# dfdazac/grapes

Measured on AMD Instinct MI355X. Metric: sampled edges aggregated/sec, ogbn-products 3-layer GFlowNet, higher is better.
Workload: dtype f32

## Files before the change

### grapes_amd/_lib.py

```python
from __future__ import annotations

import ctypes as C
import os

_HERE = os.path.dirname(os.path.abspath(__file__))
DIAG_LIB_PATH = os.path.join(_HERE, "libgrapes_hip_diag.so")
DIAG = os.environ.get("GRAPES_DIAG", "0") == "1"
LIB_PATH = os.environ.get("GRAPES_LIB_PATH") or (DIAG_LIB_PATH if DIAG else os.path.join(_HERE, "libgrapes_hip.so"))
ABI_MAJOR, ABI_MINOR = 3, 2


def diag_switch(name: str, default: str) -> str:
    if os.environ.get("GRAPES_DIAG", "0") == "1":
        return os.environ.get(name, default)
    return default


P = C.c_void_p
I32 = C.c_int32
I64 = C.c_int64
U32 = C.c_uint32
U64 = C.c_uint64
F32 = C.c_float
SZ = C.c_size_t
# ... 66 lines not shown
    "grapes_frontier_offsets": (I32, [P, P, I32, P, P, P, P]),
    "grapes_frontier_expand": (I32, [P, P, P, I32, P, P, I32, P, P, P, P, P]),
    "grapes_frontier_expand_fused": (I32, [P, P, P, I32, P, I32, P, P, P, P, P, P, P, I32, P, P, P, P, P]),
    "grapes_frontier_expand_fused_ext": (I32, [P, P, P, I32, P, I32, P, P, P, P, P, P, P, I32, P, P, P, P, P, P, P, P, P]),
    "grapes_slice_stage_words": (SZ, [I32]),
    "grapes_bitmap_mark": (I32, [P, P, P, I64, P, I32, P, P]),
    "grapes_bitmap_mark_rows": (I32, [P, P, P, I32, P, P, I32, P, P]),
    "grapes_bitmap_clear": (I32, [P, P, I64, P, P]),
    "grapes_frontier_compact_workspace_bytes": (SZ, [I32, I32]),
    "grapes_frontier_compact": (I32, [P, P, P, I32, I32, P, P, P, P, P, P, U32, P, I32, P, P, SZ, P, SZ, P, SZ, P, P, P, P, P]),
    "grapes_frontier_compact_counted": (I32, [P, P, P, I32, I32, P, P, P, P, P, P, U32, P, I32, P, P, SZ, P, SZ, P, SZ, P, P, P, P, P, P]),
    "grapes_gcn_prepare_counted": (I32, [P, P, P, I32, P, P, I32, P, P, P, P, P, P, P, P, P, P, P, P, P, I64, I32, P, P]),
    "grapes_bitmap_mark_hop": (I32, [P, P, P, P, I32, P, P, P, I32, P, I32, P, P]),
    "grapes_bitmap_mark_lists": (I32, [P, P, P, I32, P, P, I32, P, P, I32, P, P, I32, P, I32, P, P, P]),
    "grapes_union_sorted": (I32, [P, I32, P, P, I32, P, P, I32, P, P, I32, P, I32, I32, P, P, P, P, P, P]),
    "grapes_slice_mark": (I32, [P, P, I32, P, I32, P, P]),
    "grapes_slice_remark": (I32, [P, P, I32, P, P, I32, P, P, P, I32, P, P]),
    "grapes_slice_filter_workspace_bytes": (SZ, [I32]),
    "grapes_slice_filter": (I32, [P, P, P, I32, P, I32, P, P, P, P, P, I32, P, P]),
    "grapes_indicator_mark": (I32, [P, P, I32, P, U32, P, I32, I32, P]),
    "grapes_step_begin": (I32, [P, P, I32, P, I32, P, I32, I32, I32, P, P, I32, I32, P, P]),
    "grapes_gather_rows": (I32, [P, I32, P, I32, P, P, U32, P, I32, P, P]),
    "grapes_gcn_prepare_workspace_bytes": (SZ, [I32, I32]),
    "grapes_gcn_prepare_zero_words": (SZ, [I32]),
    "grapes_gcn_long_items_capacity": (I32, [I32]),
    "grapes_gcn_prepare": (I32, [P, P, I32, P, P, I32, P, I32, P, P, P, P, P, P, P, P, P, P, P, P, P]),
    "grapes_gcn_prepare_prefetching": (I32, [P, P, I32, P, P, I32, P, I32, P, P, P, P, P, P, P, P, P, P, P, P, P, I64, I32, P]),
    "grapes_gcn_prepare_small_batch": (I32, [I32, P, P, P, P, P, I32, P, P, P, P, P, P, P, P, P, P, P, P, P, P, P, P]),
    "grapes_gcn_prepare_from_csr": (I32, [P, I32, P, P, P, I32, P]),
    "grapes_linear_fwd": (I32, [P, P, P, I32, P, I32, I32, P]),
# ... 143 lines not shown
```

### grapes_amd/csrc/index_kernels.hip

```cpp
#include "common.h"

__global__ void tensormap_update_k(int32_t* __restrict__ map, const int32_t* __restrict__ keys,
                                   int n_host, const int32_t* d_n) {
    const int n = eff_count(d_n, n_host);
    for (int i = blockIdx.x * blockDim.x + threadIdx.x; i < n; i += gridDim.x * blockDim.x)
        map[keys[i]] = i;
}

__global__ void tensormap_map_k(const int32_t* __restrict__ map, const int32_t* __restrict__ keys,
                                int32_t* __restrict__ out, int64_t n_host, const int32_t* d_n) {
    int64_t n = n_host;
    if (d_n) { int64_t v = *d_n; n = v < n_host ? v : n_host; }
    for (int64_t i = (int64_t)blockIdx.x * blockDim.x + threadIdx.x; i < n;
         i += (int64_t)gridDim.x * blockDim.x)
        out[i] = map[keys[i]];
}

extern "C" int grapes_tensormap_update(int32_t* map, const int32_t* keys, int32_t n,
                                       const int32_t* d_n, grapes_stream_t stream) {
    if (!map || (!keys && n > 0) || n < 0) return GRAPES_EINVAL;
    if (n == 0) return 0;
    int grid = grapes_div_up(n, 256); if (grid > 2048) grid = 2048;
    hipLaunchKernelGGL(tensormap_update_k, dim3(grid), dim3(256), 0, (hipStream_t)stream, map, keys, n, d_n);
    GRAPES_LAUNCH_CHECK();
// ... 703 lines not shown
    bool overflow = false;
    for (int i = lo; i < hi; ++i) {
        const int v = key[i];
        if (v != 0x7fffffff && (i == 0 || key[i - 1] != v)) {
            if (pos < n_cap) { out_ids[pos] = v; if (node_map) node_map[v] = pos; }
            else overflow = true;
            if (unmark_mult) unmark_mult[v] = 0;
            ++pos;
        }
    }
    if (tid == 0) { counts[0] = tot < n_cap ? tot : n_cap; counts[1] = counts[0]; }
    if (overflow && status) atomicOr(status, GRAPES_STATUS_NODE_OVERFLOW);
    (void)s_total;
}

__global__ __launch_bounds__(1024) void union_sorted_k(MarkLists L, int num_nodes, int n_cap, int32_t* __restrict__ out_ids,
                                                       int32_t* __restrict__ node_map, int32_t* __restrict__ counts,
                                                       int32_t* __restrict__ unmark_mult, int32_t* status) {
    union_sorted_body(L, num_nodes, n_cap, out_ids, node_map, counts, unmark_mult, status);
}

extern "C" int grapes_bitmap_clear(uint64_t* bits, const int32_t* ids, int64_t n, const int32_t* d_n,
                                   grapes_stream_t stream) {
    if (!bits || (!ids && n > 0) || n < 0) return GRAPES_EINVAL;
    if (n == 0) return 0;
    int grid = grapes_div_up(n, 256); if (grid > 4096) grid = 4096;
    hipLaunchKernelGGL(bitmap_clear_k, dim3(grid), dim3(256), 0, (hipStream_t)stream,
                       (unsigned long long*)bits, ids, n, d_n);
    GRAPES_LAUNCH_CHECK();
    return 0;
}

__device__ __forceinline__ int block_prefix_of_sums(const int32_t* __restrict__ bsum, int b, int* lds) {
    int acc = 0;
// ... 252 lines not shown
};
#define COMPACT_EMIT_CALL(A, bid, nblk)                                                                                              \
    compact_emit_body((A).bits, (A).prev_bits, (A).W, (A).bsum_b, (A).bsum_n, (A).n_cap, (A).batch_nodes, (A).neighbor_nodes,          \
                      (A).nb_local, (A).node_map, (A).counts, (A).status, (A).ind_code, (A).epoch_host, (A).d_epoch, (A).ind_bit,      \
                      (A).sync, (A).cand_pos, (A).zero_a, (A).words_a, (A).zero_b, (A).words_b, (A).zero_c, (A).words_c, (A).rm,       \
                      (A).gc, (A).hd, bid, nblk)
__global__ __launch_bounds__(1024) void compact_emit_k(CompactEmitArgs a) { COMPACT_EMIT_CALL(a, (int)blockIdx.x, (int)gridDim.x); }
__global__ __launch_bounds__(1024) void compact_emit_pair_k(CompactEmitArgs a, CompactEmitArgs b, int nA) {
    if ((int)blockIdx.x < nA) COMPACT_EMIT_CALL(a, (int)blockIdx.x, nA);
    else COMPACT_EMIT_CALL(b, (int)blockIdx.x - nA, (int)gridDim.x - nA);
}

__global__ __launch_bounds__(1024) void union_sorted_compact_pair_k(MarkLists L, int num_nodes, int n_cap, int32_t* __restrict__ out_ids,
                                                                   int32_t* __restrict__ node_map, int32_t* __restrict__ counts,
                                                                   int32_t* __restrict__ unmark_mult, int32_t* status,
                                                                   CompactEmitArgs b) {
    if (blockIdx.x == 0) union_sorted_body(L, num_nodes, n_cap, out_ids, node_map, counts, unmark_mult, status);
    else COMPACT_EMIT_CALL(b, (int)blockIdx.x - 1, (int)gridDim.x - 1);
}

extern "C" int grapes_union_sorted(const int32_t* ids0, int32_t n0, const int32_t* d_n0, const int32_t* ids1, int32_t n1,
                                   const int32_t* d_n1, const int32_t* ids2, int32_t n2, const int32_t* d_n2,
                                   const int32_t* ids3, int32_t n3, const int32_t* d_n3, int32_t num_nodes, int32_t n_cap,
                                   int32_t* out_ids, int32_t* node_map, int32_t* counts, int32_t* unmark_mult,
                                   int32_t* status, grapes_stream_t stream) {
    if (n0 < 0 || n1 < 0 || n2 < 0 || n3 < 0 || num_nodes <= 0 || n_cap <= 0 || !out_ids || !counts) return GRAPES_EINVAL;
    if ((long long)n0 + n1 + n2 + n3 > UNION_MAX) return GRAPES_EINVAL;
    MarkLists L{{n0 > 0 ? ids0 : nullptr, n1 > 0 ? ids1 : nullptr, n2 > 0 ? ids2 : nullptr, n3 > 0 ? ids3 : nullptr},
                {n0, n1, n2, n3}, {d_n0, d_n1, d_n2, d_n3}};
    if (const GrapesRiderRecord* r = grapes_rider_match(GRAPES_RK_COMPACT, 0, 1024, (hipStream_t)stream)) {
        CompactEmitArgs Bq; memcpy(&Bq, r->args, sizeof Bq);
        hipLaunchKernelGGL(union_sorted_compact_pair_k, dim3(1 + r->grid), dim3(1024), 0, (hipStream_t)stream, L, num_nodes, n_cap, out_ids,
                           node_map, counts, unmark_mult, status, Bq);
    } else {
        hipLaunchKernelGGL(union_sorted_k, dim3(1), dim3(1024), 0, (hipStream_t)stream, L, num_nodes, n_cap, out_ids, node_map, counts,
                           unmark_mult, status);
    }
    GRAPES_LAUNCH_CHECK();
    return 0;
}


template <int WPT>
__global__ __launch_bounds__(1024) void compact_emit_wide_k(unsigned long long* __restrict__ bits,
                                                            const unsigned long long* __restrict__ prev_bits, int W,
                                                            int n_cap, int32_t* __restrict__ batch_nodes,
                                                            int32_t* __restrict__ neighbor_nodes, int32_t* __restrict__ nb_local,
                                                            int32_t* __restrict__ node_map, int32_t* __restrict__ counts,
                                                            int32_t* status, uint32_t* __restrict__ ind_code,
                                                            uint32_t epoch_host, const uint32_t* d_epoch, int ind_bit,
                                                            unsigned long long* __restrict__ sync, int32_t* __restrict__ cand_pos,
                                                            uint32_t* __restrict__ zero_a, size_t words_a,
                                                            uint32_t* __restrict__ zero_b, size_t words_b,
                                                            uint32_t* __restrict__ zero_c, size_t words_c,
// ... 793 lines not shown
```

### grapes_amd/csrc/prep_kernels.hip

```cpp
#include "common.h"

struct PrefetchRows { const float* X; long long pitch; int row_floats; const int32_t* ids; int32_t* sink; };
__device__ __forceinline__ void prefetch_rows_body(const PrefetchRows& pf, int n, int block, int nblocks) {
    const int spr = (pf.row_floats * 4 + 63) / 64;
    const long long total = (long long)n * spr;
    unsigned acc = 0u;
    for (long long i = (long long)block * blockDim.x + threadIdx.x; i < total; i += (long long)nblocks * blockDim.x) {
        const int r = (int)(i / spr), k = (int)(i - (long long)r * spr);
        int c = 16 * k; if (c > pf.row_floats - 1) c = pf.row_floats - 1;
        acc += __float_as_uint(pf.X[(long long)pf.ids[r] * pf.pitch + c]);
    }
    if (acc == 0x7fc12345u && pf.sink) *pf.sink = 1;
}


__global__ void prep_hist_k(const int32_t* __restrict__ es, const int32_t* __restrict__ ed, int e_host,
                            const int32_t* d_e, int n_host, const int32_t* d_n, int grouped,
                            int32_t* __restrict__ cnt_t, int32_t* __restrict__ cnt_s,
                            int32_t* __restrict__ seg_first, int32_t* __restrict__ seg_last,
                            int32_t* __restrict__ loops, int32_t* __restrict__ nseg, int32_t* __restrict__ bad,
                            int32_t* status, const int32_t* __restrict__ relabel, int32_t* __restrict__ n_long,
                            int ge, PrefetchRows pf) {
    const int e = eff_count(d_e, e_host);
    const int n = eff_count(d_n, n_host);
// ... 504 lines not shown
                            int32_t* __restrict__ rl_dst, int32_t* __restrict__ counters, size_t counter_words,
                            int32_t* __restrict__ csr_dst, int clear_dst, int32_t* __restrict__ n_long) {
    const int e = eff_count(d_e, e_host);
    if (n_long && blockIdx.x == 0 && threadIdx.x < 2) n_long[threadIdx.x] = 0;
    const size_t stride = (size_t)gridDim.x * blockDim.x;
    const size_t i0 = (size_t)blockIdx.x * blockDim.x + threadIdx.x;
    for (size_t i = i0; i < counter_words; i += stride) counters[i] = 0;
    for (size_t t = i0; t < (size_t)e_host; t += stride) {
        if (clear_dst) csr_dst[t] = 0;
        if (node_map && t < (size_t)e) { rl_src[t] = node_map[es[t]]; rl_dst[t] = node_map[ed[t]]; }
    }
}

#define SMALL_N 2048
#define SMALL_T 1024
__device__ __forceinline__ int slice_assemble(const int32_t* __restrict__ stage, int fe_cap, const int32_t* d_fe, int out_cap,
                                              int32_t* __restrict__ out_src, int32_t* __restrict__ out_dst, int32_t* d_out_count,
                                              int32_t* status, int* lds) {
    const int tid = threadIdx.x;
    const int fe = eff_count(d_fe, fe_cap);
    const int nwb_cap = (fe_cap + 63) >> 6, nwb = (fe + 63) >> 6;
    const int32_t* wcnt = stage; const int32_t* wsum = stage + nwb_cap;
    const int32_t* st_s = stage + 2 * nwb_cap; const int32_t* st_d = st_s + fe_cap; const int32_t* st_c = st_d + fe_cap;
    const int per = (nwb + SMALL_T - 1) / SMALL_T;
    const int w0 = tid * per;
    int mine = 0;
    for (int k = 0; k < per; ++k) { const int wb = w0 + k; if (wb < nwb) mine += wsum[wb]; }
    int tot;
    int pos = block_excl_scan(mine, lds, &tot);
    bool overflow = false;
    if (mine > 0) {
        for (int k = 0; k < per; ++k) {
            const int wb = w0 + k;
            if (wb >= nwb) break;
            const int cnt = wcnt[wb];
            for (int i = 0; i < cnt; ++i) {
                const int q = wb * 64 + i;
                const int sv = st_s[q], dv = st_d[q], c = st_c[q];
                for (int r = 0; r < c; ++r, ++pos) {
                    if (pos < out_cap) { out_src[pos] = sv; out_dst[pos] = dv; }
                    else overflow = true;
                }
            }
        }
    }
    if (overflow && status) atomicOr(status, GRAPES_STATUS_EDGE_OVERFLOW);
    const int total = tot < out_cap ? tot : out_cap;
    if (tid == 0 && d_out_count) *d_out_count = total;
    __syncthreads();
    return total;
}

__device__ __forceinline__ void prep_small_body(const int32_t* __restrict__ es, const int32_t* __restrict__ ed,
                                                int e_host, const int32_t* d_e, int n_host, const int32_t* d_n,
                                                const int32_t* __restrict__ node_map,
                                                int32_t* __restrict__ rowptr_t, int32_t* __restrict__ csr_src,
                                                int32_t* __restrict__ rowptr_s, int32_t* __restrict__ csr_dst,
                                                float* __restrict__ dinv, int32_t* __restrict__ long_items,
                                                int32_t* __restrict__ n_long, int item_cap,
                                                int32_t* __restrict__ tmp_src, int32_t* status,
                                                const int32_t* __restrict__ head_ids,
                                                int32_t* __restrict__ row_head, const int32_t* __restrict__ slice_stage = nullptr,
                                                int fe_cap = 0, const int32_t* d_fe = nullptr) {
    __shared__ int cnt_t[SMALL_N], segf[SMALL_N], segl[SMALL_N], loops[SMALL_N], nseg[SMALL_N], rps[SMALL_N];
    __shared__ int lds[17];
    __shared__ int s_bad, s_nlong_rows;
    __shared__ int long_rows[SMALL_N];
    const int tid = threadIdx.x;
    const int e = slice_stage ? slice_assemble(slice_stage, fe_cap, d_fe, e_host, const_cast<int32_t*>(es), const_cast<int32_t*>(ed),
                                               const_cast<int32_t*>(d_e), status, lds)
                              : eff_count(d_e, e_host);
    const int n = eff_count(d_n, n_host);
    for (int i = tid; i < n; i += SMALL_T) { cnt_t[i] = 0; loops[i] = 0; nseg[i] = 0; }
    if (tid == 0) { s_bad = 0; s_nlong_rows = 0; if (n_long) { n_long[0] = 0; n_long[1] = 0; } }
    constexpr int EPT = 2;
    int c_gs[EPT], c_s[EPT], c_d[EPT], c_pv[EPT], c_nx[EPT];
    int r_gd[EPT];
#pragma unroll
    for (int k = 0; k < EPT; ++k) { c_gs[k] = 0; c_pv[k] = 0; c_nx[k] = 0; r_gd[k] = 0; }
    if (e_host > 0) {
#pragma unroll
        for (int k = 0; k < EPT; ++k) {
            const int t = tid + k * SMALL_T;
            const int tc = t < e ? t : 0;
            const int tp = tc > 0 ? tc - 1 : 0, tn = tc + 1 < e ? tc + 1 : tc;
            c_gs[k] = es[tc]; c_pv[k] = es[tp]; c_nx[k] = es[tn]; r_gd[k] = ed[tc];
// ... 3 lines not shown
    for (int k = 0; k < EPT; ++k) {
        const int t = tid + k * SMALL_T;
        const int tc = t < e ? t : 0;
        c_gs[k] = e > 0 ? c_gs[k] : 0;
        c_pv[k] = (e > 0 && tc > 0) ? c_pv[k] : -1;
        c_nx[k] = (e > 0 && tc + 1 < e) ? c_nx[k] : -1;
        r_gd[k] = e > 0 ? r_gd[k] : 0;
    }
    if (node_map) {
#pragma unroll
        for (int k = 0; k < EPT; ++k) { c_s[k] = node_map[c_gs[k]]; c_d[k] = node_map[r_gd[k]]; }
    } else {
#pragma unroll
        for (int k = 0; k < EPT; ++k) { c_s[k] = c_gs[k]; c_d[k] = r_gd[k]; }
    }
    __syncthreads();
    for (int t = tid; t < e; t += SMALL_T) {
        csr_dst[t] = 0;
        const int kk = (t - tid) / SMALL_T;
        int gs, s, d;
        if (kk < EPT) { gs = kk == 0 ? c_gs[0] : c_gs[1]; s = kk == 0 ? c_s[0] : c_s[1]; d = kk == 0 ? c_d[0] : c_d[1]; }
        else { gs = es[t]; s = node_map ? node_map[gs] : gs; d = node_map ? node_map[ed[t]] : ed[t]; }
        if ((unsigned)s >= (unsigned)n || (unsigned)d >= (unsigned)n) {
            if (status) atomicOr(status, GRAPES_STATUS_BAD_INDEX);
            continue;
        }
        const int pv = kk < EPT ? (kk == 0 ? c_pv[0] : c_pv[1]) : (t > 0 ? es[t - 1] : -1);
        const int nx = kk < EPT ? (kk == 0 ? c_nx[0] : c_nx[1]) : (t + 1 < e ? es[t + 1] : -1);
        if (t == 0 || pv != gs) {
            segf[s] = t;
            if (atomicAdd(&nseg[s], 1) > 0) { s_bad = 1; if (status) atomicOr(status, GRAPES_STATUS_BAD_INDEX); }
        }
        if (t == e - 1 || nx != gs) segl[s] = t;
        if (s == d) { atomicAdd(&loops[s], 1); continue; }
        atomicAdd(&cnt_t[d], 1);
    }
    __syncthreads();
    const int isbad = s_bad;
    const int i0 = 2 * tid, i1 = 2 * tid + 1;
    int ct0 = 0, ct1 = 0, cs0 = 0, cs1 = 0;
    if (i0 < n) { ct0 = cnt_t[i0]; if (!isbad && nseg[i0] > 0) { const int v = segl[i0] - segf[i0] + 1 - loops[i0]; cs0 = v > 0 ? v : 0; } }
    if (i1 < n) { ct1 = cnt_t[i1]; if (!isbad && nseg[i1] > 0) { const int v = segl[i1] - segf[i1] + 1 - loops[i1]; cs1 = v > 0 ? v : 0; } }
    int tt, ts;
    const int pt = block_excl_scan(ct0 + ct1, lds, &tt);
    const int ps = block_excl_scan(cs0 + cs1, lds, &ts);
    __syncthreads();
#pragma unroll
    for (int k = 0; k < 2; ++k) {
        const int i = k ? i1 : i0;
        if (i >= n) continue;
        const int ct = k ? ct1 : ct0, cs = k ? cs1 : cs0;
        const int bt = k ? pt + ct0 : pt, bs = k ? ps + cs0 : ps;
// ... 6 lines not shown
                const int nc = (ct + GRAPES_LONG_ROW - 1) / GRAPES_LONG_ROW;
                const int b = atomicAdd(&n_long[0], nc);
                for (int c = 0; c < nc; ++c)
                    if (b + c < item_cap) { long_items[2 * (b + c)] = i; long_items[2 * (b + c) + 1] = c; }
            }
            if (cs > GRAPES_LONG_ROW) {
                const int nc = (cs + GRAPES_LONG_ROW - 1) / GRAPES_LONG_ROW;
                const int b = atomicAdd(&n_long[1], nc);
                for (int c = 0; c < nc; ++c)
                    if (b + c < item_cap) { long_items[2 * (item_cap + b + c)] = i; long_items[2 * (item_cap + b + c) + 1] = c; }
            }
        }
    }
    if (tid == 0) { rowptr_t[n] = tt; rowptr_s[n] = ts; if (n_long) n_long[2] = tt; }
    __syncthreads();
    for (int t = tid; t < e; t += SMALL_T) {
        const int kk = (t - tid) / SMALL_T;
        int s, d;
        if (kk < EPT) { s = kk == 0 ? c_s[0] : c_s[1]; d = kk == 0 ? c_d[0] : c_d[1]; }
        else { const int gs = es[t]; s = node_map ? node_map[gs] : gs; d = node_map ? node_map[ed[t]] : ed[t]; }
        if ((unsigned)s >= (unsigned)n || (unsigned)d >= (unsigned)n || s == d) continue;
        tmp_src[atomicAdd(&cnt_t[d], 1)] = s;
        if (!isbad) {
            const int p = rps[s] + (t - segf[s]) - (d > s ? loops[s] : 0);
            if ((unsigned)p < (unsigned)e_host) csr_dst[p] = d;
            else if (status) atomicOr(status, GRAPES_STATUS_BAD_INDEX);
        }
    }
    __threadfence_block();
    __syncthreads();
#pragma unroll
    for (int k = 0; k < 2; ++k) {
        const int i = k ? i1 : i0;
        const int len = i < n ? (k ? ct1 : ct0) : 0;
        if (len > 0 && len <= SORT_SHORT) {
            const int beg = k ? pt + ct0 : pt;
            int v[SORT_SHORT];
#pragma unroll
            for (int q = 0; q < SORT_SHORT; ++q) v[q] = q < len ? tmp_src[beg + q] : 0x7fffffff;
#pragma unroll
            for (int q = 1; q < SORT_SHORT; ++q) {
#pragma unroll
                for (int j = q; j > 0; --j) {
                    const int a = v[j - 1], b = v[j];
                    v[j - 1] = a < b ? a : b;
// ... 22 lines not shown
    const int lane = lane_id(), wid = tid >> 6;
    for (int q = wid; q < nl; q += SMALL_T / 64) {
        const int r = long_rows[q];
        const int beg = rowptr_t[r], len = rowptr_t[r + 1] - beg;
        for (int i = lane; i < len; i += 64) {
            const int v = tmp_src[beg + i];
            int rank = 0;
            for (int j = 0; j < len; ++j) {
                const int u = tmp_src[beg + j];
                rank += (u < v) || (u == v && j < i);
            }
            csr_src[beg + rank] = v;
            if (row_head && rank < HEAD_ENTRIES) head_write_entry(row_head, head_ids, dinv, r, rank, v);
        }
    }
}

__global__ __launch_bounds__(SMALL_T) void prep_small_k(const int32_t* es, const int32_t* ed, int e_host, const int32_t* d_e,
                                                        int n_host, const int32_t* d_n, const int32_t* node_map,
                                                        int32_t* rowptr_t, int32_t* csr_src, int32_t* rowptr_s,
                                                        int32_t* csr_dst, float* dinv, int32_t* long_items, int32_t* n_long,
                                                        int item_cap, int32_t* tmp_src, int32_t* status,
                                                        const int32_t* head_ids, int32_t* row_head) {
    prep_small_body(es, ed, e_host, d_e, n_host, d_n, node_map, rowptr_t, csr_src, rowptr_s, csr_dst, dinv, long_items, n_long,
                    item_cap, tmp_src, status, head_ids, row_head);
}

#define SMALL_BATCH_MAX 8
struct SmallGraph {
    const int32_t* es; const int32_t* ed; const int32_t* d_e; int e_host;
// ... 308 lines not shown
```

### grapes_amd/ops.py

```python
from __future__ import annotations

from typing import List, Optional

import os

import torch

from . import _lib
from ._lib import diag_switch as _sw

_i32 = torch.int32
_i64 = torch.int64
_f32 = torch.float32


def lib():
    return _lib.load()


def _stream() -> int:
    try:
        return torch._C._cuda_getCurrentRawStream(torch._C._cuda_getDevice())
    except AttributeError:
        return torch.cuda.current_stream().cuda_stream
# ... 284 lines not shown
               "bitmap_mark_hop")


def bitmap_mark_lists(bits, bits1, lists, num_nodes, status=None, unmark_mult=None):
    _chk(bits, _i64, "bits"); _chk(bits1, _i64, "bits1", True); _chk(unmark_mult, _i32, "unmark_mult", True)
    if len(lists) > 4:
        raise ValueError("at most four lists per launch")
    args = []
    for ids, d_n in list(lists) + [(None, None)] * (4 - len(lists)):
        _chk(ids, _i32, "ids", True)
        args += [_p(ids), 0 if ids is None else ids.numel(), _p(d_n)]
    _lib.check(lib().grapes_bitmap_mark_lists(_p(bits), _p(bits1), *args, num_nodes, _p(status), _p(unmark_mult), _stream()),
               "bitmap_mark_lists")


def union_sorted(lists, num_nodes, n_cap, node_map=None, status=None, unmark_mult=None):
    if not (1 <= len(lists) <= 4) or sum(ids.numel() for ids, _ in lists) > 4096:
        raise ValueError("union_sorted: 1..4 lists, at most 4096 ids in all")
    _chk(node_map, _i32, "node_map", True); _chk(unmark_mult, _i32, "unmark_mult", True)
    dev = lists[0][0].device
    args = []
    for ids, d_n in list(lists) + [(None, None)] * (4 - len(lists)):
        _chk(ids, _i32, "ids", True)
        args += [_p(ids), 0 if ids is None else ids.numel(), _p(d_n)]
    out = torch.empty(n_cap, dtype=_i32, device=dev)
    counts = torch.empty(2, dtype=_i32, device=dev)
    _lib.check(lib().grapes_union_sorted(*args, num_nodes, n_cap, _p(out), _p(node_map), _p(counts), _p(unmark_mult), _p(status),
                                         _stream()), "union_sorted")
    return out, counts


def frontier_compact(bits, bits1, prev_bits, num_nodes, n_cap, node_map=None, status=None, ind_code=None, epoch=0,
                     d_epoch=None, ind_bit=0, sync=None, one_launch=True, want_cand_pos=False, zero=(), remark=None,
                     degrees=None):
    _chk(ind_code, _i32, "ind_code", True)
    _chk(bits, _i64, "bits"); _chk(bits1, _i64, "bits1", True); _chk(prev_bits, _i64, "prev_bits", True)
    _chk(node_map, _i32, "node_map", True)
    dev = bits.device
    batch = torch.empty(n_cap, dtype=_i32, device=dev)
    neigh = torch.empty(n_cap, dtype=_i32, device=dev)
    nbl = torch.empty(n_cap, dtype=_i32, device=dev)
# ... 1674 lines not shown
```

### grapes_amd/step_graph.py

```python
from __future__ import annotations

import contextlib
from typing import Dict, List, Optional

import os

import torch

from ._lib import diag_switch as _sw
import torch.nn as nn

from . import ops
from .capture import SegmentedGraph
from .graph import DeviceGraph


class _FirstLayer:

    def __init__(self, conv, F, num_ind, legacy=False):
        self.conv, self.F, self.num_ind = conv, F, num_ind
        self.K = F + num_ind
        self.Kp = self.K if legacy else (self.K + 3) // 4 * 4
        self.agg_first = legacy or self.K < conv.out_channels or conv.out_channels % 4 != 0
        self.padded = self.Kp != self.K
# ... 579 lines not shown
                src, dst, d_e, eoff = self._expand(batch_next, d_m_next, mark=hop + 1 < hops, prev_buf=cur_prev)
            if staged:
                kcap = min(e_cap, (B + K) * (B + K))
                ksrc = torch.empty(kcap, dtype=torch.int32, device=targets.device)
                kdst = torch.empty(kcap, dtype=torch.int32, device=targets.device)
                kcnt = torch.empty(1, dtype=torch.int32, device=targets.device)
                stages.append((sstage, d_e, e_cap))
            elif ev:
                ksrc, kdst, kcnt = ev_slice
            else:
                ksrc, kdst, kcnt = ops.slice_filter(g.mult, src, dst, min(e_cap, (B + K) * (B + K)), d_e=d_e, status=st,
                                                    bsum=bsum if fused else None)
            slices.append((ksrc, kdst, kcnt))
            previous, d_m = batch_next, d_m_next
        marks = [(targets, None)] + [(kept, cnt) for kept, cnt in kept_list]
        if len(marks) <= 4 and sum(m_[0].numel() for m_ in marks) <= 4096:
            alln, counts = ops.union_sorted(marks, N, self.nall_cap, node_map=g.node_map, status=st, unmark_mult=None if ev else g.mult)
        else:
            for i in range(0, len(marks), 4):
                ops.bitmap_mark_lists(g.bits, g.bits1, marks[i:i + 4], N, status=st, unmark_mult=g.mult)
            alln, _, _, counts = ops.frontier_compact(g.bits, g.bits1, None, N, self.nall_cap, node_map=g.node_map,
                                                      status=st)
        d_na = counts[0:1]
        hid = None if self.partitioned else alln
        if self.nall_cap <= 2048 and len(slices) <= 8:
            preps = ops.PreparedGraph.small_batch(slices, self.nall_cap, d_n=d_na, status=st, node_map=g.node_map,
                                                  head_ids=hid, counters=ctr[hops:], stages=stages if staged else None)
        else:
            preps = [ops.PreparedGraph(ksrc, kdst, self.nall_cap, d_n=d_na, d_e=kcnt, status=st, src_grouped=True,
                                       node_map=g.node_map, head_ids=hid, counters=ctr[hops + i])
                     for i, (ksrc, kdst, kcnt) in enumerate(slices)]
        layers = list(self.gcn_c.gcn_layers)
        used = [preps[-i] for i in range(1, len(layers))] + [preps[0]]
        first_relu = len(layers) > 1
        first_fused = (not self.partitioned) or (len(layers) > 1 and self.F < layers[0].out_channels)
        pdrop = self.dropout
        keeps: List[Optional[torch.Tensor]] = []

        def drop(t):
            if not pdrop:
                keeps.append(None)
                return t
# ... 503 lines not shown
```

### include/grapes_hip.h

```cpp
#ifndef GRAPES_HIP_H
#define GRAPES_HIP_H

#include <stddef.h>
#include <stdint.h>

#ifdef __cplusplus
extern "C" {
#endif

#define GRAPES_ABI_VERSION 302

#define GRAPES_EINVAL (-1)
#define GRAPES_EALIGN (-2)

#define GRAPES_STATUS_EDGE_OVERFLOW 1
#define GRAPES_STATUS_NODE_OVERFLOW 2
#define GRAPES_STATUS_BAD_INDEX 4
#define GRAPES_STATUS_SYNC_TIMEOUT 8
#define GRAPES_SYNC_WORDS 256

typedef void* grapes_stream_t;

int grapes_abi_version(void);
const char* grapes_target_arch(void);
// ... 88 lines not shown
                               int32_t* cursor, grapes_stream_t stream);

int grapes_bitmap_mark_hop(uint64_t* prev_bits, uint64_t* bits, uint64_t* bits1, const int32_t* previous,
                           int32_t m, const int32_t* d_m, const int32_t* eoff, const int32_t* dst, int32_t e,
                           const int32_t* d_e, int32_t num_nodes, int32_t* status, grapes_stream_t stream);
int grapes_bitmap_mark_lists(uint64_t* bits, uint64_t* bits1, const int32_t* ids0, int32_t n0,
                             const int32_t* d_n0, const int32_t* ids1, int32_t n1, const int32_t* d_n1,
                             const int32_t* ids2, int32_t n2, const int32_t* d_n2, const int32_t* ids3,
                             int32_t n3, const int32_t* d_n3, int32_t num_nodes, int32_t* status,
                             int32_t* unmark_mult, grapes_stream_t stream);

int grapes_union_sorted(const int32_t* ids0, int32_t n0, const int32_t* d_n0, const int32_t* ids1, int32_t n1,
                        const int32_t* d_n1, const int32_t* ids2, int32_t n2, const int32_t* d_n2, const int32_t* ids3,
                        int32_t n3, const int32_t* d_n3, int32_t num_nodes, int32_t n_cap, int32_t* out_ids,
                        int32_t* node_map, int32_t* counts, int32_t* unmark_mult, int32_t* status, grapes_stream_t stream);

int grapes_slice_mark(int32_t* mult, const int32_t* cols, int32_t c, const int32_t* d_c,
                      int32_t unmark, uint64_t* clear_bits, grapes_stream_t stream);
int grapes_slice_remark(int32_t* mult, const int32_t* unmark_ids, int32_t n_unmark, const int32_t* d_n_unmark,
                        const int32_t* mark_ids, int32_t n_mark, const int32_t* d_n_mark, uint64_t* clear_bits,
                        const int32_t* clear_ids, int32_t n_clear, const int32_t* d_n_clear, grapes_stream_t stream);
size_t grapes_slice_filter_workspace_bytes(int32_t e_cap);
int grapes_slice_filter(const int32_t* mult, const int32_t* src, const int32_t* dst, int32_t e,
                        const int32_t* d_e, int32_t out_cap, int32_t* out_src, int32_t* out_dst,
                        int32_t* d_out_count, void* workspace, uint64_t* sync, int32_t counted, int32_t* status,
                        grapes_stream_t stream);

int grapes_indicator_mark(uint32_t* ind_code, const int32_t* ids, int32_t n, const int32_t* d_n,
                          uint32_t epoch, uint32_t* d_epoch, int32_t bit, int32_t advance_epoch,
                          grapes_stream_t stream);
// ... 430 lines not shown
```

Baseline: 505.5 million.

## Fold staged edge-list assembly into union_sorted launch across wide workgroups

Edge-list assembly from the staged slice buffers moves out of the single-workgroup small-batch GCN prep kernel. It now runs as extra workgroups attached to the union_sorted launch, with each graph's block range split across up to 32 workgroups using wave-level scans and readlane-driven copies. The intent is to take the serial per-graph assembly off the prep kernel's critical path and run it in parallel with the node union. The cost is a more complex launch and per-block prefix recomputation over the preceding block sums. Optional timestamp instrumentation, off by default, is also added along with a profiling script.

```diff
diff --git a/grapes_amd/_lib.py b/grapes_amd/_lib.py
--- a/grapes_amd/_lib.py
+++ b/grapes_amd/_lib.py
@@ -104,6 +104,8 @@
     "grapes_bitmap_mark_hop": (I32, [P, P, P, P, I32, P, P, P, I32, P, I32, P, P]),
     "grapes_bitmap_mark_lists": (I32, [P, P, P, I32, P, P, I32, P, P, I32, P, P, I32, P, I32, P, P, P]),
     "grapes_union_sorted": (I32, [P, I32, P, P, I32, P, P, I32, P, P, I32, P, I32, I32, P, P, P, P, P, P]),
+    "grapes_union_sorted_assemble": (I32, [P, I32, P, P, I32, P, P, I32, P, P, I32, P, I32, I32, P, P, P, P, I32, P, P, P, P, P, P, P,
+                                           P, P]),
     "grapes_slice_mark": (I32, [P, P, I32, P, I32, P, P]),
     "grapes_slice_remark": (I32, [P, P, I32, P, P, I32, P, P, P, I32, P, P]),
     "grapes_slice_filter_workspace_bytes": (SZ, [I32]),
diff --git a/grapes_amd/csrc/index_kernels.hip b/grapes_amd/csrc/index_kernels.hip
--- a/grapes_amd/csrc/index_kernels.hip
+++ b/grapes_amd/csrc/index_kernels.hip
@@ -741,10 +741,19 @@
     (void)s_total;
 }
 
+#define SLICE_WIDE_MAX 8
+#define SLICE_WIDE_G 32
+struct SliceWideGraph {
+    const int32_t* stage; const int32_t* d_fe; int fe_cap; int out_cap; int32_t* out_src; int32_t* out_dst; int32_t* d_out_count;
+};
+struct SliceWideArgs { int count; int G; SliceWideGraph g[SLICE_WIDE_MAX]; };
+__device__ __forceinline__ void slice_assemble_wide(const SliceWideGraph& g, int j, int G, int32_t* status);
+
 __global__ __launch_bounds__(1024) void union_sorted_k(MarkLists L, int num_nodes, int n_cap, int32_t* __restrict__ out_ids,
                                                        int32_t* __restrict__ node_map, int32_t* __restrict__ counts,
-                                                       int32_t* __restrict__ unmark_mult, int32_t* status) {
-    union_sorted_body(L, num_nodes, n_cap, out_ids, node_map, counts, unmark_mult, status);
+                                                       int32_t* __restrict__ unmark_mult, int32_t* status, SliceWideArgs sw) {
+    if (blockIdx.x == 0) union_sorted_body(L, num_nodes, n_cap, out_ids, node_map, counts, unmark_mult, status);
+    else { const int a = (int)blockIdx.x - 1; slice_assemble_wide(sw.g[a / sw.G], a % sw.G, sw.G, status); }
 }
 
 extern "C" int grapes_bitmap_clear(uint64_t* bits, const int32_t* ids, int64_t n, const int32_t* d_n,
@@ -1027,9 +1036,32 @@
 __global__ __launch_bounds__(1024) void union_sorted_compact_pair_k(MarkLists L, int num_nodes, int n_cap, int32_t* __restrict__ out_ids,
                                                                    int32_t* __restrict__ node_map, int32_t* __restrict__ counts,
                                                                    int32_t* __restrict__ unmark_mult, int32_t* status,
-                                                                   CompactEmitArgs b) {
+                                                                   CompactEmitArgs b, int nB, SliceWideArgs sw) {
     if (blockIdx.x == 0) union_sorted_body(L, num_nodes, n_cap, out_ids, node_map, counts, unmark_mult, status);
-    else COMPACT_EMIT_CALL(b, (int)blockIdx.x - 1, (int)gridDim.x - 1);
+    else if ((int)blockIdx.x <= nB) COMPACT_EMIT_CALL(b, (int)blockIdx.x - 1, nB);
+    else { const int a = (int)blockIdx.x - 1 - nB; slice_assemble_wide(sw.g[a / sw.G], a % sw.G, sw.G, status); }
+}
+
+static int union_sorted_launch(const int32_t* ids0, int32_t n0, const int32_t* d_n0, const int32_t* ids1, int32_t n1,
+                               const int32_t* d_n1, const int32_t* ids2, int32_t n2, const int32_t* d_n2,
+                               const int32_t* ids3, int32_t n3, const int32_t* d_n3, int32_t num_nodes, int32_t n_cap,
+                               int32_t* out_ids, int32_t* node_map, int32_t* counts, int32_t* unmark_mult,
+                               int32_t* status, const SliceWideArgs& sw, grapes_stream_t stream) {
+    if (n0 < 0 || n1 < 0 || n2 < 0 || n3 < 0 || num_nodes <= 0 || n_cap <= 0 || !out_ids || !counts) return GRAPES_EINVAL;
+    if ((long long)n0 + n1 + n2 + n3 > UNION_MAX) return GRAPES_EINVAL;
+    MarkLists L{{n0 > 0 ? ids0 : nullptr, n1 > 0 ? ids1 : nullptr, n2 > 0 ? ids2 : nullptr, n3 > 0 ? ids3 : nullptr},
+                {n0, n1, n2, n3}, {d_n0, d_n1, d_n2, d_n3}};
+    const int na = sw.count * sw.G;
+    if (const GrapesRiderRecord* r = grapes_rider_match(GRAPES_RK_COMPACT, 0, 1024, (hipStream_t)stream)) {
+        CompactEmitArgs Bq; memcpy(&Bq, r->args, sizeof Bq);
+        hipLaunchKernelGGL(union_sorted_compact_pair_k, dim3(1 + r->grid + na), dim3(1024), 0, (hipStream_t)stream, L, num_nodes, n_cap,
+                           out_ids, node_map, counts, unmark_mult, status, Bq, (int)r->grid, sw);
+    } else {
+        hipLaunchKernelGGL(union_sorted_k, dim3(1 + na), dim3(1024), 0, (hipStream_t)stream, L, num_nodes, n_cap, out_ids, node_map, counts,
+                           unmark_mult, status, sw);
+    }
+    GRAPES_LAUNCH_CHECK();
+    return 0;
 }
 
 extern "C" int grapes_union_sorted(const int32_t* ids0, int32_t n0, const int32_t* d_n0, const int32_t* ids1, int32_t n1,
@@ -1037,20 +1069,34 @@
                                    const int32_t* ids3, int32_t n3, const int32_t* d_n3, int32_t num_nodes, int32_t n_cap,
                                    int32_t* out_ids, int32_t* node_map, int32_t* counts, int32_t* unmark_mult,
                                    int32_t* status, grapes_stream_t stream) {
-    if (n0 < 0 || n1 < 0 || n2 < 0 || n3 < 0 || num_nodes <= 0 || n_cap <= 0 || !out_ids || !counts) return GRAPES_EINVAL;
-    if ((long long)n0 + n1 + n2 + n3 > UNION_MAX) return GRAPES_EINVAL;
-    MarkLists L{{n0 > 0 ? ids0 : nullptr, n1 > 0 ? ids1 : nullptr, n2 > 0 ? ids2 : nullptr, n3 > 0 ? ids3 : nullptr},
-                {n0, n1, n2, n3}, {d_n0, d_n1, d_n2, d_n3}};
-    if (const GrapesRiderRecord* r = grapes_rider_match(GRAPES_RK_COMPACT, 0, 1024, (hipStream_t)stream)) {
-        CompactEmitArgs Bq; memcpy(&Bq, r->args, sizeof Bq);
-        hipLaunchKernelGGL(union_sorted_compact_pair_k, dim3(1 + r->grid), dim3(1024), 0, (hipStream_t)stream, L, num_nodes, n_cap, out_ids,
-                           node_map, counts, unmark_mult, status, Bq);
-    } else {
-        hipLaunchKernelGGL(union_sorted_k, dim3(1), dim3(1024), 0, (hipStream_t)stream, L, num_nodes, n_cap, out_ids, node_map, counts,
-                           unmark_mult, status);
-    }
-    GRAPES_LAUNCH_CHECK();
-    return 0;
+    SliceWideArgs sw; memset(&sw, 0, sizeof sw); sw.G = 1;
+    return union_sorted_launch(ids0, n0, d_n0, ids1, n1, d_n1, ids2, n2, d_n2, ids3, n3, d_n3, num_nodes, n_cap, out_ids, node_map,
+                               counts, unmark_mult, status, sw, stream);
+}
+
+extern "C" int grapes_union_sorted_assemble(const int32_t* ids0, int32_t n0, const int32_t* d_n0, const int32_t* ids1, int32_t n1,
+                                            const int32_t* d_n1, const int32_t* ids2, int32_t n2, const int32_t* d_n2,
+                                            const int32_t* ids3, int32_t n3, const int32_t* d_n3, int32_t num_nodes, int32_t n_cap,
+                                            int32_t* out_ids, int32_t* node_map, int32_t* counts, int32_t* unmark_mult,
+                                            int32_t count, const int32_t* const* slice_stage, const int32_t* const* d_fe,
+                                            const int32_t* fe_cap, const int32_t* out_cap, int32_t* const* out_src,
+                                            int32_t* const* out_dst, int32_t* const* out_count, int32_t* status,
+                                            grapes_stream_t stream) {
+    if (count < 1 || count > SLICE_WIDE_MAX || !slice_stage || !d_fe || !fe_cap || !out_cap || !out_src || !out_dst || !out_count)
+        return GRAPES_EINVAL;
+    SliceWideArgs sw; memset(&sw, 0, sizeof sw);
+    sw.count = count; sw.G = 1;
+    for (int i = 0; i < count; ++i) {
+        if (!slice_stage[i] || fe_cap[i] <= 0 || out_cap[i] <= 0 || !out_src[i] || !out_dst[i] || !out_count[i]) return GRAPES_EINVAL;
+        const int nwb_cap = (fe_cap[i] + 63) / 64;
+        if (nwb_cap > SLICE_WIDE_G * 1024) return GRAPES_EINVAL;
+        int G = grapes_div_up(nwb_cap, 64); if (G > SLICE_WIDE_G) G = SLICE_WIDE_G;
+        if (G > sw.G) sw.G = G;
+        sw.g[i] = SliceWideGraph{slice_stage[i], d_fe[i], fe_cap[i], out_cap[i], out_src[i], out_dst[i], out_count[i]};
+    }
+    for (int i = count; i < SLICE_WIDE_MAX; ++i) sw.g[i] = sw.g[0];
+    return union_sorted_launch(ids0, n0, d_n0, ids1, n1, d_n1, ids2, n2, d_n2, ids3, n3, d_n3, num_nodes, n_cap, out_ids, node_map,
+                               counts, unmark_mult, status, sw, stream);
 }
 
 
diff --git a/grapes_amd/csrc/prep_kernels.hip b/grapes_amd/csrc/prep_kernels.hip
--- a/grapes_amd/csrc/prep_kernels.hip
+++ b/grapes_amd/csrc/prep_kernels.hip
@@ -542,6 +542,19 @@
 
 #define SMALL_N 2048
 #define SMALL_T 1024
+#ifdef GRAPES_STAMPS
+static __device__ unsigned long long* prep_stamp_ptr = nullptr;
+#define PREP_STAMP(slot)                                                                                     \
+    do {                                                                                                     \
+        if (prep_stamp_ptr && threadIdx.x == 0 && blockIdx.x < 8) {                                          \
+            asm volatile("s_waitcnt vmcnt(0) lgkmcnt(0)" ::: "memory");                                      \
+            prep_stamp_ptr[blockIdx.x * 16 + (slot)] = wall_clock64();                                        \
+        }                                                                                                    \
+    } while (0)
+extern "C" int grapes_stamp_set_prep(unsigned long long* p) { return (int)hipMemcpyToSymbol(HIP_SYMBOL(prep_stamp_ptr), &p, sizeof(p)); }
+#else
+#define PREP_STAMP(slot) do { } while (0)
+#endif
 __device__ __forceinline__ int slice_assemble(const int32_t* __restrict__ stage, int fe_cap, const int32_t* d_fe, int out_cap,
                                               int32_t* __restrict__ out_src, int32_t* __restrict__ out_dst, int32_t* d_out_count,
                                               int32_t* status, int* lds) {
@@ -554,8 +567,10 @@
     const int w0 = tid * per;
     int mine = 0;
     for (int k = 0; k < per; ++k) { const int wb = w0 + k; if (wb < nwb) mine += wsum[wb]; }
+    PREP_STAMP(8);
     int tot;
     int pos = block_excl_scan(mine, lds, &tot);
+    PREP_STAMP(9);
     bool overflow = false;
     if (mine > 0) {
         for (int k = 0; k < per; ++k) {
@@ -572,11 +587,81 @@
             }
         }
     }
+    PREP_STAMP(10);
     if (overflow && status) atomicOr(status, GRAPES_STATUS_EDGE_OVERFLOW);
     const int total = tot < out_cap ? tot : out_cap;
     if (tid == 0 && d_out_count) *d_out_count = total;
     __syncthreads();
     return total;
+}
+
+__device__ __forceinline__ void slice_assemble_wide(const SliceWideGraph& g, int j, int G, int32_t* status) {
+    __shared__ int sw_bef[SMALL_T / 64], sw_own[SMALL_T / 64];
+    const int tid = threadIdx.x, lane = tid & 63, wid = tid >> 6;
+    const int fe_cap = g.fe_cap, out_cap = g.out_cap;
+    const int fe = eff_count(g.d_fe, fe_cap);
+    const int nwb_cap = (fe_cap + 63) >> 6, nwb = (fe + 63) >> 6;
+    const int32_t* __restrict__ wcnt = g.stage; const int32_t* __restrict__ wsum = g.stage + nwb_cap;
+    const int32_t* __restrict__ st_s = g.stage + 2 * nwb_cap; const int32_t* __restrict__ st_d = st_s + fe_cap;
+    const int32_t* __restrict__ st_c = st_d + fe_cap;
+    int32_t* __restrict__ out_src = g.out_src; int32_t* __restrict__ out_dst = g.out_dst;
+    const int share = (nwb + G - 1) / G;
+    const int b0 = j * share < nwb ? j * share : nwb, b1 = b0 + share < nwb ? b0 + share : nwb;
+    const int cpw = (share + SMALL_T / 64 - 1) / (SMALL_T / 64);
+    const int blk = b0 + wid * cpw + lane;
+    const bool have = lane < cpw && blk < b1;
+    const int own_raw = wsum[have ? blk : 0], cnt_raw = wcnt[have ? blk : 0];
+    const int lim = j == 0 ? nwb : b0;
+    int bef = 0;
+    for (int i0 = tid; i0 < lim + tid; i0 += 4 * SMALL_T) {
+        int v[4];
+#pragma unroll
+        for (int k = 0; k < 4; ++k) { const int i = i0 + k * SMALL_T; v[k] = wsum[i < lim ? i : 0]; }
+#pragma unroll
+        for (int k = 0; k < 4; ++k) bef += (i0 + k * SMALL_T < lim) ? v[k] : 0;
+    }
+    const int own = have ? own_raw : 0;
+    int cnt = have ? cnt_raw : 0;
+    cnt = cnt < 0 ? 0 : (cnt > 64 ? 64 : cnt);
+    const int own_incl = wave_incl_scan(own), bef_incl = wave_incl_scan(bef);
+    if (lane == 63) { sw_own[wid] = own_incl; sw_bef[wid] = bef_incl; }
+    __syncthreads();
+    int front = 0, sum_bef = 0;
+#pragma unroll
+    for (int u = 0; u < SMALL_T / 64; ++u) { sum_bef += sw_bef[u]; front += u < wid ? sw_own[u] : 0; }
+    const int pos = (j == 0 ? 0 : sum_bef) + front + own_incl - own;
+    if (j == 0 && tid == 0 && g.d_out_count) *g.d_out_count = sum_bef < out_cap ? sum_bef : out_cap;
+    bool overflow = false;
+    unsigned long long m = __ballot(have && cnt > 0);
+    while (m != 0ull) {
+        int bb[4], bc[4], bp[4];
+#pragma unroll
+        for (int k = 0; k < 4; ++k) {
+            if (m != 0ull) {
+                const int l = __builtin_amdgcn_readfirstlane((int)__ffsll((long long)m) - 1);
+                m &= m - 1;
+                bb[k] = __builtin_amdgcn_readlane(blk, l); bc[k] = __builtin_amdgcn_readlane(cnt, l); bp[k] = __builtin_amdgcn_readlane(pos, l);
+            } else { bb[k] = bb[0]; bc[k] = 0; bp[k] = 0; }
+        }
+        int sv[4], dv[4], cv[4];
+#pragma unroll
+        for (int k = 0; k < 4; ++k) {
+            int q = bb[k] * 64 + (lane < bc[k] ? lane : 0);
+            q = q < fe_cap ? q : 0;
+            sv[k] = st_s[q]; dv[k] = st_d[q]; cv[k] = st_c[q];
+        }
+#pragma unroll
+        for (int k = 0; k < 4; ++k) {
+            int c = lane < bc[k] ? cv[k] : 0;
+            c = c < 0 ? 0 : c;
+            int p = bp[k] + wave_incl_scan(c) - c;
+            for (int r = 0; r < c; ++r, ++p) {
+                if ((unsigned)p < (unsigned)out_cap) { out_src[p] = sv[k]; out_dst[p] = dv[k]; }
+                else overflow = true;
+            }
+        }
+    }
+    if (overflow && status) atomicOr(status, GRAPES_STATUS_EDGE_OVERFLOW);
 }
 
 __device__ __forceinline__ void prep_small_body(const int32_t* __restrict__ es, const int32_t* __restrict__ ed,
@@ -595,9 +680,11 @@
     __shared__ int s_bad, s_nlong_rows;
     __shared__ int long_rows[SMALL_N];
     const int tid = threadIdx.x;
+    PREP_STAMP(0);
     const int e = slice_stage ? slice_assemble(slice_stage, fe_cap, d_fe, e_host, const_cast<int32_t*>(es), const_cast<int32_t*>(ed),
                                                const_cast<int32_t*>(d_e), status, lds)
                               : eff_count(d_e, e_host);
+    PREP_STAMP(1);
     const int n = eff_count(d_n, n_host);
     for (int i = tid; i < n; i += SMALL_T) { cnt_t[i] = 0; loops[i] = 0; nseg[i] = 0; }
     if (tid == 0) { s_bad = 0; s_nlong_rows = 0; if (n_long) { n_long[0] = 0; n_long[1] = 0; } }
@@ -631,6 +718,7 @@
 #pragma unroll
         for (int k = 0; k < EPT; ++k) { c_s[k] = c_gs[k]; c_d[k] = r_gd[k]; }
     }
+    PREP_STAMP(2);
     __syncthreads();
     for (int t = tid; t < e; t += SMALL_T) {
         csr_dst[t] = 0;
@@ -653,6 +741,7 @@
         atomicAdd(&cnt_t[d], 1);
     }
     __syncthreads();
+    PREP_STAMP(3);
     const int isbad = s_bad;
     const int i0 = 2 * tid, i1 = 2 * tid + 1;
     int ct0 = 0, ct1 = 0, cs0 = 0, cs1 = 0;
@@ -689,6 +778,7 @@
     }
     if (tid == 0) { rowptr_t[n] = tt; rowptr_s[n] = ts; if (n_long) n_long[2] = tt; }
     __syncthreads();
+    PREP_STAMP(4);
     for (int t = tid; t < e; t += SMALL_T) {
         const int kk = (t - tid) / SMALL_T;
         int s, d;
@@ -704,6 +794,7 @@
     }
     __threadfence_block();
     __syncthreads();
+    PREP_STAMP(5);
 #pragma unroll
     for (int k = 0; k < 2; ++k) {
         const int i = k ? i1 : i0;
@@ -756,6 +847,7 @@
             if (row_head && rank < HEAD_ENTRIES) head_write_entry(row_head, head_ids, dinv, r, rank, v);
         }
     }
+    PREP_STAMP(6);
 }
 
 __global__ __launch_bounds__(SMALL_T) void prep_small_k(const int32_t* es, const int32_t* ed, int e_host, const int32_t* d_e,
diff --git a/grapes_amd/ops.py b/grapes_amd/ops.py
--- a/grapes_amd/ops.py
+++ b/grapes_amd/ops.py
@@ -322,7 +322,10 @@
                "bitmap_mark_lists")
 
 
-def union_sorted(lists, num_nodes, n_cap, node_map=None, status=None, unmark_mult=None):
+SLICE_WIDE_FE_CAP = 1 << 21
+
+
+def union_sorted(lists, num_nodes, n_cap, node_map=None, status=None, unmark_mult=None, assemble=None):
     if not (1 <= len(lists) <= 4) or sum(ids.numel() for ids, _ in lists) > 4096:
         raise ValueError("union_sorted: 1..4 lists, at most 4096 ids in all")
     _chk(node_map, _i32, "node_map", True); _chk(unmark_mult, _i32, "unmark_mult", True)
@@ -333,6 +336,25 @@
         args += [_p(ids), 0 if ids is None else ids.numel(), _p(d_n)]
     out = torch.empty(n_cap, dtype=_i32, device=dev)
     counts = torch.empty(2, dtype=_i32, device=dev)
+    if assemble:
+        import ctypes as C
+        k = len(assemble)
+        if k > 8:
+            raise ValueError("union_sorted: at most 8 edge lists to assemble")
+        for stage, d_fe, fe_cap, osrc, odst, ocnt in assemble:
+            _chk(stage, _i32, "slice_stage"); _chk(d_fe, _i32, "d_fe", True); _chk(osrc, _i32, "out_src"); _chk(odst, _i32, "out_dst")
+            _chk(ocnt, _i32, "out_count")
+            if not (0 < int(fe_cap) <= SLICE_WIDE_FE_CAP) or stage.numel() < int(lib().grapes_slice_stage_words(int(fe_cap))):
+                raise ValueError("union_sorted: a stage of grapes_slice_stage_words(fe_cap) words, 0 < fe_cap <= 2^21")
+            if osrc.numel() < 1 or odst.numel() < osrc.numel() or ocnt.numel() < 1:
+                raise ValueError("union_sorted: out_src / out_dst of one capacity >= 1, out_count of one word")
+        arr = lambda ts: (C.c_void_p * k)(*[None if t is None else t.data_ptr() for t in ts])
+        _lib.check(lib().grapes_union_sorted_assemble(
+            *args, num_nodes, n_cap, _p(out), _p(node_map), _p(counts), _p(unmark_mult), k, arr([a[0] for a in assemble]),
+            arr([a[1] for a in assemble]), (C.c_int32 * k)(*[int(a[2]) for a in assemble]),
+            (C.c_int32 * k)(*[a[3].numel() for a in assemble]), arr([a[3] for a in assemble]), arr([a[4] for a in assemble]),
+            arr([a[5] for a in assemble]), _p(status), _stream()), "union_sorted_assemble")
+        return out, counts
     _lib.check(lib().grapes_union_sorted(*args, num_nodes, n_cap, _p(out), _p(node_map), _p(counts), _p(unmark_mult), _p(status),
                                          _stream()), "union_sorted")
     return out, counts
diff --git a/grapes_amd/step_graph.py b/grapes_amd/step_graph.py
--- a/grapes_amd/step_graph.py
+++ b/grapes_amd/step_graph.py
@@ -617,8 +617,13 @@
             slices.append((ksrc, kdst, kcnt))
             previous, d_m = batch_next, d_m_next
         marks = [(targets, None)] + [(kept, cnt) for kept, cnt in kept_list]
+        wide = False
         if len(marks) <= 4 and sum(m_[0].numel() for m_ in marks) <= 4096:
-            alln, counts = ops.union_sorted(marks, N, self.nall_cap, node_map=g.node_map, status=st, unmark_mult=None if ev else g.mult)
+            wide = (staged and self.nall_cap <= 2048 and len(slices) <= 8 and e_cap <= ops.SLICE_WIDE_FE_CAP
+                    and _sw("GRAPES_SLICE_WIDE", "1") != "0")
+            alln, counts = ops.union_sorted(marks, N, self.nall_cap, node_map=g.node_map, status=st, unmark_mult=None if ev else g.mult,
+                                            assemble=[(sg, dfe, cap, sl[0], sl[1], sl[2]) for (sg, dfe, cap), sl in zip(stages, slices)]
+                                            if wide else None)
         else:
             for i in range(0, len(marks), 4):
                 ops.bitmap_mark_lists(g.bits, g.bits1, marks[i:i + 4], N, status=st, unmark_mult=g.mult)
@@ -628,7 +633,7 @@
         hid = None if self.partitioned else alln
         if self.nall_cap <= 2048 and len(slices) <= 8:
             preps = ops.PreparedGraph.small_batch(slices, self.nall_cap, d_n=d_na, status=st, node_map=g.node_map,
-                                                  head_ids=hid, counters=ctr[hops:], stages=stages if staged else None)
+                                                  head_ids=hid, counters=ctr[hops:], stages=stages if (staged and not wide) else None)
         else:
             preps = [ops.PreparedGraph(ksrc, kdst, self.nall_cap, d_n=d_na, d_e=kcnt, status=st, src_grouped=True,
                                        node_map=g.node_map, head_ids=hid, counters=ctr[hops + i])
diff --git a/include/grapes_hip.h b/include/grapes_hip.h
--- a/include/grapes_hip.h
+++ b/include/grapes_hip.h
@@ -126,6 +126,14 @@
                         const int32_t* d_n1, const int32_t* ids2, int32_t n2, const int32_t* d_n2, const int32_t* ids3,
                         int32_t n3, const int32_t* d_n3, int32_t num_nodes, int32_t n_cap, int32_t* out_ids,
                         int32_t* node_map, int32_t* counts, int32_t* unmark_mult, int32_t* status, grapes_stream_t stream);
+
+int grapes_union_sorted_assemble(const int32_t* ids0, int32_t n0, const int32_t* d_n0, const int32_t* ids1, int32_t n1,
+                                 const int32_t* d_n1, const int32_t* ids2, int32_t n2, const int32_t* d_n2,
+                                 const int32_t* ids3, int32_t n3, const int32_t* d_n3, int32_t num_nodes, int32_t n_cap,
+                                 int32_t* out_ids, int32_t* node_map, int32_t* counts, int32_t* unmark_mult, int32_t count,
+                                 const int32_t* const* slice_stage, const int32_t* const* d_fe, const int32_t* fe_cap,
+                                 const int32_t* out_cap, int32_t* const* out_src, int32_t* const* out_dst,
+                                 int32_t* const* out_count, int32_t* status, grapes_stream_t stream);
 
 int grapes_slice_mark(int32_t* mult, const int32_t* cols, int32_t c, const int32_t* d_c,
                       int32_t unmark, uint64_t* clear_bits, grapes_stream_t stream);
diff --git a/profiles/classifier_build_stamps.py b/profiles/classifier_build_stamps.py
--- /dev/null
+++ b/profiles/classifier_build_stamps.py
@@ -0,0 +1,70 @@
+#!/usr/bin/env python3
+import argparse, ctypes, os, sys
+import numpy as np, torch
+ROOT = os.path.dirname(os.path.dirname(os.path.abspath(__file__)))
+sys.path.insert(0, ROOT)
+ap = argparse.ArgumentParser()
+ap.add_argument("--workload", default="products")
+ap.add_argument("--batches", type=int, default=24)
+pa = ap.parse_args()
+sys.argv = [sys.argv[0], "--workload", pa.workload]
+import bench
+from grapes_amd import ops, _lib
+lib = _lib.load()
+lib.grapes_stamp_set_prep.argtypes = [ctypes.c_void_p]
+dev = torch.device("cuda", 0)
+args = bench.parse()
+b = bench.Bench(args, 1, 0, dev)
+tr, g, models = b.make("single", capture=False, pipeline=False)
+tr.attach_loader(b.train_idx, stride=1, offset=0)
+for _ in range(4):
+    tr.step_next()
+torch.cuda.synchronize()
+us = 1e6 / (lib.grapes_kernel_clock_rate_khz() * 1e3)
+buf = torch.zeros(8 * 16, dtype=torch.int64, device=dev)
+assert lib.grapes_stamp_set_prep(buf.data_ptr()) == 0
+tabs, staged_calls = [], []
+orig = ops.PreparedGraph.small_batch.__func__
+
+
+def small_batch(cls, *a, **k):
+    torch.cuda.synchronize()
+    buf.zero_()
+    torch.cuda.synchronize()
+    r = orig(cls, *a, **k)
+    torch.cuda.synchronize()
+    tabs.append(buf.cpu().numpy().reshape(8, 16).astype(np.float64).copy())
+    staged_calls.append(k.get("stages") is not None)
+    return r
+
+
+ops.PreparedGraph.small_batch = classmethod(small_batch)
+for _ in range(pa.batches):
+    tr.step_next()
+torch.cuda.synchronize()
+tr.check()
+WHAT = [(0, "start"), (8, "assembly: live count + block sums arrived"), (9, "assembly: workgroup scan done"),
+        (10, "assembly: thread 0's entries copied"), (1, "edge list there (assembled and barrier passed / count read)"),
+        (2, "first two edges' ids + relabels arrived"), (3, "pass 1 done"), (4, "scan done, row pointers / dinv written"),
+        (5, "pass 2 done"), (6, "rows ordered, head records written (end)")]
+st = np.stack(tabs[2:])
+print(f"# workload {pa.workload}; prep_small_batch_k, {st.shape[0]} eager launches of the real step (first two dropped); "
+      f"edge lists assembled inside the build: {all(staged_calls)}")
+live = st[:, :, 0] > 0
+t0 = np.where(live, st[:, :, 0], np.inf).min(axis=1)
+for wg in range(8):
+    if not live[:, wg].any():
+        continue
+    print(f"workgroup {wg} (graph {wg})")
+    for sl, what in WHAT:
+        ok = live[:, wg] & (st[:, wg, sl] > 0)
+        if not ok.any():
+            print(f"   [{sl:2d}] {what:64s} (not on this path)")
+            continue
+        d = (st[ok, wg, sl] - t0[ok]) * us
+        print(f"   [{sl:2d}] {what:64s} median {np.median(d):6.2f} us   p10 {np.percentile(d, 10):6.2f}   p90 {np.percentile(d, 90):6.2f}")
+asm = (st[:, :, 1] - st[:, :, 0])[live] * us
+end = np.where(live, st[:, :, 6], -np.inf).max(axis=1) - t0
+print(f"start -> edge list there, all stamped workgroups: median {np.median(asm):.2f} us, max-over-workgroups median "
+      f"{np.median(np.where(live, st[:, :, 1] - st[:, :, 0], -np.inf).max(axis=1) * us):.2f} us")
+print(f"span, earliest start -> latest end: median {np.median(end * us):.2f} us")
```

New measurement: 509.4 million, median of 6. About the same (+0.8%).
